# ecmwf/earthkit-meteo

Measured on NVIDIA B200. Metric: thermo grid-points/s, higher is better.
Workload: dtype f64

## Files before the change

### earthkit-meteo_b200/csrc/ek_api.cu

```cuda
#include <cstring>
#include <vector>

#include "ek_launch.cuh"

namespace ek {

std::atomic<int> g_ctas_per_sm{16};
std::atomic<uint64_t> g_launches{0};

static thread_local char t_err[512] = "";

int set_error(int code, const char* fmt, ...) {
    va_list ap;
    va_start(ap, fmt);
    vsnprintf(t_err, sizeof(t_err), fmt, ap);
    va_end(ap);
    return code;
}

int sm_count_current_device() {
    static std::atomic<int> cache[64];
    int dev = -1;
    if (cudaGetDevice(&dev) != cudaSuccess || dev < 0) return -1;
    if (dev < 64) {
        int v = cache[dev].load(std::memory_order_relaxed);
        if (v > 0) return v;
    }
    int sms = 0;
    if (cudaDeviceGetAttribute(&sms, cudaDevAttrMultiProcessorCount, dev) != cudaSuccess) return -1;
    if (dev < 64) cache[dev].store(sms, std::memory_order_relaxed);
    return sms;
}

}

using namespace ek;

extern "C" EK_EXPORT int ek_thermo_version(void) { return EK_THERMO_VERSION; }
extern "C" EK_EXPORT const char* ek_thermo_last_error(void) { return t_err; }
extern "C" EK_EXPORT uint64_t ek_thermo_launch_count(void) { return g_launches.load(std::memory_order_relaxed); }

extern "C" EK_EXPORT int ek_thermo_set_launch_config(int threads, int ctas_per_sm) {
    if (threads != 0 && threads != kThreads) return set_error(EK_ERR_ARG, "threads=%d: the CTA size is fixed at build time (%d)", threads, kThreads);
    if (ctas_per_sm != 0) {
        if (ctas_per_sm < 1 || ctas_per_sm > 4096) return set_error(EK_ERR_ARG, "ctas_per_sm=%d out of range", ctas_per_sm);
        g_ctas_per_sm.store(ctas_per_sm);
    }
    return EK_OK;
}

extern "C" EK_EXPORT int ek_thermo_shard_range(int64_t n, int world, int rank, int64_t align, int64_t* begin, int64_t* end) {
    if (n < 0 || world < 1 || rank < 0 || rank >= world || align < 1 || !begin || !end)
        return set_error(EK_ERR_ARG, "shard_range: bad arguments n=%lld world=%d rank=%d align=%lld", (long long)n, world, rank, (long long)align);
    const int64_t units = n / align;
    const int64_t base = units / world, extra = units % world;
    const int64_t b = (rank * base + (rank < extra ? rank : extra)) * align;
    int64_t e = b + (base + (rank < extra ? 1 : 0)) * align;
    if (rank == world - 1) e = n;
    *begin = b;
    *end = e;
    return EK_OK;
}

template <typename T> int ek_suite_launch_tqp(const ek_operand* ins, void* const* outs, uint32_t mask, int ept_method, int64_t n, void* stream);
template <typename T> int ek_suite_launch_ttdp(const ek_operand* ins, void* const* outs, uint32_t mask, int ept_method, int64_t n, void* stream);
template <typename T>
int ek_suite_launch_hybrid(const void* t, const void* q, const void* sp, const void* A, const void* B, int nlev, int64_t npl, void* const* outs,
                           uint32_t out_mask, int ept_method, void* stream);

namespace {
struct StreamSet {
    std::vector<cudaStream_t> s;
    ~StreamSet() {
        for (auto st : s) cudaStreamSynchronize(st);
        for (auto st : s) cudaStreamDestroy(st);
    }
    int create(int n) {
        for (int i = 0; i < n; ++i) {
            cudaStream_t st;
            cudaError_t e = cudaStreamCreateWithFlags(&st, cudaStreamNonBlocking);
            if (e != cudaSuccess) return set_error((int)e, "host pipeline: cudaStreamCreate: %s", cudaGetErrorString(e));
            s.push_back(st);
        }
        return EK_OK;
    }
    int drain() {
        for (auto st : s) {
            cudaError_t e = cudaStreamSynchronize(st);
            if (e != cudaSuccess) return set_error((int)e, "host pipeline: stream sync: %s", cudaGetErrorString(e));
        }
        return EK_OK;
    }
};

int count_outputs(const char* what, void* const* h_outs, uint32_t out_mask, int* n_out) {
    if (out_mask == 0 || out_mask >= (1u << S_NSLOTS)) return set_error(EK_ERR_ARG, "%s: out_mask=0x%x", what, out_mask);
    *n_out = 0;
    for (int k = 0; k < S_NSLOTS; ++k)
        if ((out_mask >> k) & 1u) {
            if (!h_outs[k]) return set_error(EK_ERR_ARG, "%s: output %d requested but its buffer is NULL", what, k);
// ... 132 lines not shown
```

### earthkit-meteo_b200/csrc/ek_launch.cuh

```cuda
#pragma once
#include <atomic>
#include <cstdarg>
#include <cstdio>

#include "../../include/ek_thermo.h"
#include "ek_thermo_kernels.cuh"

#define EK_EXPORT __attribute__((visibility("default")))

#ifndef EK_SMALL_WAVE_SPARE
#define EK_SMALL_WAVE_SPARE 0
#endif

namespace ek {

int set_error(int code, const char* fmt, ...);
int sm_count_current_device();
extern std::atomic<int> g_ctas_per_sm;
extern std::atomic<uint64_t> g_launches;

inline bool aligned16(const void* p) { return (reinterpret_cast<uintptr_t>(p) & 15u) == 0; }

template <typename T> constexpr unsigned smem_for() { return sizeof(T) == 8 ? kSmemBytes : 0u; }

template <auto Kernel> inline void prepare_smem(unsigned smem_bytes) {
    if (smem_bytes == 0) return;
    static std::atomic<uint64_t> done{0};
    int dev = 0;
    if (cudaGetDevice(&dev) != cudaSuccess || dev < 0) return;
    const uint64_t bit = dev < 64 ? (1ull << dev) : 0;
    if (bit && (done.load(std::memory_order_relaxed) & bit)) return;
    const unsigned want = EK_MIN_CTAS * (smem_bytes + 1024u);
    int pct = (int)((want * 100u + 228u * 1024u - 1u) / (228u * 1024u));
    if (pct > 100) pct = 100;
    cudaFuncSetAttribute(Kernel, cudaFuncAttributePreferredSharedMemoryCarveout, pct);
    if (smem_bytes > 48u * 1024u) cudaFuncSetAttribute(Kernel, cudaFuncAttributeMaxDynamicSharedMemorySize, (int)smem_bytes);
    if (bit) done.fetch_or(bit, std::memory_order_relaxed);
}

template <auto Kernel, typename... Args> inline void launch_kernel_smem(int blocks, cudaStream_t st, unsigned smem, Args... args) {
    prepare_smem<Kernel>(smem);
    Kernel<<<blocks, kThreads, smem, st>>>(args...);
}
template <auto Kernel, typename T, typename... Args> inline void launch_kernel(int blocks, cudaStream_t st, Args... args) {
    launch_kernel_smem<Kernel>(blocks, st, smem_for<T>(), args...);
}

template <auto Kernel, typename... Args>
inline void launch_streaming(unsigned blocks, unsigned smem, cudaStream_t st, Args... args) {
    prepare_smem<Kernel>(smem);
    cudaLaunchConfig_t cfg = {};
    cfg.gridDim = dim3(blocks);
    cfg.blockDim = dim3(kThreads);
    cfg.dynamicSmemBytes = smem;
    cfg.stream = st;
    cudaLaunchAttribute attr[1];
    attr[0].id = cudaLaunchAttributeProgrammaticStreamSerialization;
    attr[0].val.programmaticStreamSerializationAllowed = 1;
    cfg.attrs = attr;
    cfg.numAttrs = EK_PDL ? 1 : 0;
    cudaLaunchKernelEx(&cfg, Kernel, args...);
}

template <class Op, class OpE, typename T>
int launch(const char* what, const ek_operand* ins, void* const* outs, int64_t n, Params P, void* stream) {
    if (n < 0) return set_error(EK_ERR_ARG, "%s: n=%lld must be >= 0", what, (long long)n);
    InArgs<Op::NIN> in;
    OutArgs<Op::NOUT> out;
    int vec_ok = 1;
    for (int k = 0; k < Op::NIN; ++k) {
        in.p[k] = ins[k].ptr;
        in.s[k] = ins[k].value;
        if (ins[k].ptr) {
            if (!aligned16(ins[k].ptr)) vec_ok = 0;
            if (reinterpret_cast<uintptr_t>(ins[k].ptr) % sizeof(T))
                return set_error(EK_ERR_ARG, "%s: input %d is not aligned to its element size", what, k);
        }
    }
    uint32_t mask = 0;
    for (int o = 0; o < Op::NOUT; ++o) {
        out.p[o] = outs[o];
        if (outs[o]) {
            mask |= 1u << o;
            if (!aligned16(outs[o])) vec_ok = 0;
            if (reinterpret_cast<uintptr_t>(outs[o]) % sizeof(T))
                return set_error(EK_ERR_ARG, "%s: output %d is not aligned to its element size", what, o);
        }
    }
    if (mask == 0) return set_error(EK_ERR_ARG, "%s: no output buffer given", what);
    P.out_mask = mask;
    if (n == 0) return EK_OK;

    constexpr int threads = kThreads;
    constexpr int unroll = UnrollOf<Op>::value;
    const int64_t tile = (int64_t)threads * Vec16<T>::N * unroll;
    const int64_t ntiles = n / tile;
    const int64_t tail_blocks = ((n - ntiles * tile) + threads - 1) / threads;
    const int sms = sm_count_current_device();
    if (sms <= 0) return set_error(EK_ERR_ARG, "%s: no CUDA device is current", what);
    int64_t cap = (int64_t)sms * g_ctas_per_sm.load(std::memory_order_relaxed);
    const int64_t wave = (int64_t)sms * (MinCtasOf<Op>::value - EK_SMALL_WAVE_SPARE);
    if (ntiles <= 8 * wave && wave < cap) cap = wave;
    int64_t blocks = ntiles > tail_blocks ? ntiles : tail_blocks;
    if (blocks > cap) blocks = cap;
    if (blocks < 1) blocks = 1;

    launch_streaming<&ew_kernel<Op, OpE, T, unroll>>((unsigned)blocks, smem_for<T>(), static_cast<cudaStream_t>(stream), in, out, n, P, vec_ok);
    g_launches.fetch_add(1, std::memory_order_relaxed);
    cudaError_t err = cudaGetLastError();
    if (err != cudaSuccess) return set_error((int)err, "%s: kernel launch failed: %s", what, cudaGetErrorString(err));
    return EK_OK;
}

template <class Op, class OpE, typename T>
int launch_batch(const char* what, int n_seg, const void* const* const* ins, const double* scalars, const double* last_scalars,
                 void* const* const* outs, int64_t n_per_seg, Params P, void* stream) {
    if (n_seg < 0 || n_per_seg < 0) return set_error(EK_ERR_ARG, "%s: n_seg=%d n_per_seg=%lld", what, n_seg, (long long)n_per_seg);
    uint32_t in_mask = 0, out_mask = 0;
    for (int k = 0; k < Op::NIN; ++k)
        if (ins[k]) in_mask |= 1u << k;
    for (int o = 0; o < Op::NOUT; ++o)
        if (outs[o]) out_mask |= 1u << o;
    if (out_mask == 0) return set_error(EK_ERR_ARG, "%s: no output buffer given", what);
    if (last_scalars && ins[Op::NIN - 1]) return set_error(EK_ERR_ARG, "%s: the last input is given both as fields and as per-segment scalars", what);
    P.out_mask = out_mask;
    if (n_seg == 0 || n_per_seg == 0) return EK_OK;
    const int sms = sm_count_current_device();
    if (sms <= 0) return set_error(EK_ERR_ARG, "%s: no CUDA device is current", what);
    constexpr int unroll = UnrollOf<Op>::value;
    const int64_t tile = (int64_t)kThreads * Vec16<T>::N * unroll;
    for (int s0 = 0; s0 < n_seg; s0 += kBatchMaxSeg) {
        BatchArgs<Op::NIN, Op::NOUT> B;
        B.n_seg = n_seg - s0 < kBatchMaxSeg ? n_seg - s0 : kBatchMaxSeg;
        B.in_mask = in_mask;
        B.out_mask = out_mask;
        B.last_per_seg = last_scalars ? 1 : 0;
        for (int j = 0; j < B.n_seg; ++j) B.s_last[j] = last_scalars ? last_scalars[s0 + j] : 0.0;
        int vec_ok = 1;
        for (int k = 0; k < Op::NIN; ++k) {
            B.s[k] = scalars ? scalars[k] : 0.0;
            for (int j = 0; j < B.n_seg; ++j) {
                B.in[k][j] = ins[k] ? ins[k][s0 + j] : nullptr;
                if (ins[k]) {
                    if (!B.in[k][j] || reinterpret_cast<uintptr_t>(B.in[k][j]) % sizeof(T))
                        return set_error(EK_ERR_ARG, "%s: input %d of segment %d is NULL or not aligned to its element size", what, k, s0 + j);
                    if (!aligned16(B.in[k][j])) vec_ok = 0;
                }
            }
        }
        for (int o = 0; o < Op::NOUT; ++o)
            for (int j = 0; j < B.n_seg; ++j) {
                B.out[o][j] = outs[o] ? outs[o][s0 + j] : nullptr;
                if (outs[o]) {
                    if (!B.out[o][j] || reinterpret_cast<uintptr_t>(B.out[o][j]) % sizeof(T))
                        return set_error(EK_ERR_ARG, "%s: output %d of segment %d is NULL or not aligned to its element size", what, o, s0 + j);
                    if (!aligned16(B.out[o][j])) vec_ok = 0;
                }
            }
        const int64_t ntiles = (n_per_seg / tile) * B.n_seg;
        const int64_t tail_blocks = ((n_per_seg % tile) * B.n_seg + kThreads - 1) / kThreads;
        int64_t cap = (int64_t)sms * g_ctas_per_sm.load(std::memory_order_relaxed);
        const int64_t wave = (int64_t)sms * MinCtasOf<Op>::value;
        if (ntiles <= 8 * wave && wave < cap) cap = wave;
        int64_t blocks = ntiles > tail_blocks ? ntiles : tail_blocks;
        if (blocks > cap) blocks = cap;
        if (blocks < 1) blocks = 1;
        launch_streaming<&ew_batch_kernel<Op, OpE, T, unroll>>((unsigned)blocks, smem_for<T>(), static_cast<cudaStream_t>(stream), B, n_per_seg, P, vec_ok);
        g_launches.fetch_add(1, std::memory_order_relaxed);
        cudaError_t err = cudaGetLastError();
        if (err != cudaSuccess) return set_error((int)err, "%s: kernel launch failed: %s", what, cudaGetErrorString(err));
    }
    return EK_OK;
}

inline bool valid_phase(int v) { return v >= 0 && v <= 2; }

#define EK_API(NAME, PARAMS, ARGS)                                                    \
    extern "C" EK_EXPORT int ek_thermo_##NAME##_f64 PARAMS { return impl_##NAME<double> ARGS; } \
    extern "C" EK_EXPORT int ek_thermo_##NAME##_f32 PARAMS { return impl_##NAME<float> ARGS; }

}
```

### earthkit-meteo_b200/csrc/ek_thermo_kernels.cuh

```cuda
#pragma once
#include <cuda_runtime.h>

#include "ek_thermo_math.cuh"

#ifndef EK_UNROLL
#define EK_UNROLL 2
#endif
#ifndef EK_PIPELINE
#define EK_PIPELINE 0
#endif
#ifndef EK_MAX_THREADS
#define EK_MAX_THREADS 256
#endif
#ifndef EK_DEFER_TILE
#define EK_DEFER_TILE 0
#endif
#ifndef EK_PF_DIST
#define EK_PF_DIST 2
#endif
#ifndef EK_HEAVY_MIN_CTAS
#define EK_HEAVY_MIN_CTAS 3
#endif
#ifndef EK_LAST_SCALAR_LOOP
#define EK_LAST_SCALAR_LOOP 1
#endif
#ifndef EK_PDL
#define EK_PDL 1
#endif
#ifndef EK_MIN_CTAS
#define EK_MIN_CTAS 4
#endif

namespace ek {

template <int N> struct InArgs {
    const void* p[N];
    double s[N];
};
template <int N> struct OutArgs {
    void* p[N];
};

template <typename T> struct Vec16;
template <> struct Vec16<double> {
    using type = double2;
    static constexpr int N = 2;
    static __device__ __forceinline__ void load(const double* src, double* dst) {
        double2 v = __ldcs(reinterpret_cast<const double2*>(src));
        dst[0] = v.x;
        dst[1] = v.y;
    }
    static __device__ __forceinline__ void store(double* dst, const double* src) {
        __stcs(reinterpret_cast<double2*>(dst), make_double2(src[0], src[1]));
    }
};
template <> struct Vec16<float> {
    using type = float4;
    static constexpr int N = 4;
    static __device__ __forceinline__ void load(const float* src, float* dst) {
        float4 v = __ldcs(reinterpret_cast<const float4*>(src));
        dst[0] = v.x;
        dst[1] = v.y;
        dst[2] = v.z;
        dst[3] = v.w;
    }
    static __device__ __forceinline__ void store(float* dst, const float* src) {
        __stcs(reinterpret_cast<float4*>(dst), make_float4(src[0], src[1], src[2], src[3]));
    }
};

#if EK_LEAN_MATH
constexpr unsigned kSmemBytes = 2 * 8 * EK_LOG_TAB_N + 8 * EK_EXP_TAB_N;
#else
constexpr unsigned kSmemBytes = 0;
#endif

constexpr int kThreads = EK_MAX_THREADS;

template <typename T> __device__ __forceinline__ bool is_nan_val(T v) { return v != v; }

template <class OpE, typename T> __device__ __noinline__ void cold_point(const T* a, T* r, const Params P, const uint32_t array_mask) {
    bool missing = array_mask != 0;
#pragma unroll
    for (int k = 0; k < OpE::NIN; ++k)
        if ((array_mask >> k) & 1u) missing = missing && is_nan_val(a[k]);
    if (missing) return;
#pragma unroll
    for (int o = 0; o < OpE::NOUT; ++o) r[o] = T(0);
    OpE::template apply<T>(a, r, P);
}

template <int NOUT> __device__ __forceinline__ bool any_nan(const double* r) {
    int m = 0;
#pragma unroll
    for (int o = 0; o < NOUT; ++o) m = max(m, __double2hiint(r[o]) & 0x7fffffff);
    return m >= 0x7ff80000;
}
template <int NOUT> __device__ __forceinline__ bool any_nan(const float* r) {
    int m = 0;
#pragma unroll
    for (int o = 0; o < NOUT; ++o) m = max(m, __float_as_int(r[o]) & 0x7fffffff);
    return m > 0x7f800000;
}

template <class Op, class = void> struct ColdF32 {
    static constexpr bool value = false;
};
template <class Op> struct ColdF32<Op, decltype((void)Op::COLD_F32)> {
    static constexpr bool value = Op::COLD_F32;
};

template <class Op, class OpE, typename T>
__device__ __forceinline__ void point(const T* a, T* r, const Params& P, const uint32_t array_mask) {
#pragma unroll
    for (int o = 0; o < Op::NOUT; ++o) r[o] = T(0);
    Op::template apply<T>(a, r, P);
#if EK_LEAN_DEVICE
    if ((sizeof(T) == 8 || ColdF32<Op>::value) && __builtin_expect(any_nan<Op::NOUT>(r), 0)) {
        T a2[Op::NIN], r2[Op::NOUT];
#pragma unroll
// ... 234 lines not shown
                } else {
#pragma unroll
                    for (int v = 0; v < VEC; ++v) __stcs(dst + v, y[o][v]);
                }
            }
        }
    }
}

template <class Op, class OpE, typename T, int UNROLL, bool VECOK, int ALLARR>
__device__ __forceinline__ void tile_loop(const InArgs<Op::NIN>& in, const OutArgs<Op::NOUT>& out, const int64_t ntiles, const Params& P,
                                          const uint32_t array_mask) {
    constexpr int TILE = kThreads * Vec16<T>::N * UNROLL;
    const int64_t G = gridDim.x;
    const int64_t toff = (int64_t)threadIdx.x * Vec16<T>::N;
    int64_t ta = blockIdx.x;
    if (ta >= ntiles) return;
#if EK_PIPELINE
    TileRegs<Op, T, UNROLL> A, B;
    load_tile<Op, T, UNROLL, VECOK, ALLARR>(A, in, ta * TILE + toff);
    for (;;) {
        const int64_t tb = ta + G;
        const bool hb = tb < ntiles;
        if (hb) load_tile<Op, T, UNROLL, VECOK, ALLARR>(B, in, tb * TILE + toff);
        compute_store_tile<Op, OpE, T, UNROLL, VECOK>(A, out, ta * TILE + toff, P, array_mask);
        if (!hb) break;
        ta = tb + G;
        const bool ha = ta < ntiles;
        if (ha) load_tile<Op, T, UNROLL, VECOK, ALLARR>(A, in, ta * TILE + toff);
        compute_store_tile<Op, OpE, T, UNROLL, VECOK>(B, out, tb * TILE + toff, P, array_mask);
        if (!ha) break;
    }
#else
    for (; ta < ntiles; ta += G) {
        TileRegs<Op, T, UNROLL> A;
        load_tile<Op, T, UNROLL, VECOK, ALLARR>(A, in, ta * TILE + toff);
        if (Op::PREFETCH_NEXT && ta + EK_PF_DIST * G < ntiles) prefetch_tile_l2<Op, T, UNROLL>(in, (ta + EK_PF_DIST * G) * TILE + toff);
        compute_store_tile<Op, OpE, T, UNROLL, VECOK>(A, out, ta * TILE + toff, P, array_mask);
    }
#endif
}

__device__ __forceinline__ void pdl_release() {
#if EK_PDL
    asm volatile("griddepcontrol.launch_dependents;");
#endif
}
__device__ __forceinline__ void pdl_acquire() {
#if EK_PDL
    asm volatile("griddepcontrol.wait;" ::: "memory");
#endif
}

template <class Op, class OpE, typename T, int UNROLL>
__global__ void __launch_bounds__(kThreads, MinCtasOf<Op>::value)
    ew_kernel(const InArgs<Op::NIN> in, const OutArgs<Op::NOUT> out, const int64_t n, const Params P, const int vec_ok) {
    constexpr int NIN = Op::NIN;
    constexpr int NOUT = Op::NOUT;
    constexpr int TILE = kThreads * Vec16<T>::N * UNROLL;
    pdl_release();
#if EK_LEAN_DEVICE
    static_assert(sizeof(lean::Tables) == kSmemBytes, "kSmemBytes must match lean::Tables");
    if (sizeof(T) == 8) lean::init_tables();
#endif
    pdl_acquire();
    const int64_t ntiles = n / TILE;
    uint32_t array_mask = 0;
#pragma unroll
    for (int k = 0; k < NIN; ++k) array_mask |= (in.p[k] != nullptr) ? (1u << k) : 0u;
    if (vec_ok && array_mask == (1u << NIN) - 1u)
        tile_loop<Op, OpE, T, UNROLL, true, 1>(in, out, ntiles, P, array_mask);
    else if (LastScalarLoopOf<Op>::value && NIN >= 2 && vec_ok && array_mask == (1u << (NIN - 1)) - 1u)
        tile_loop<Op, OpE, T, UNROLL, true, 2>(in, out, ntiles, P, array_mask);
    else if (vec_ok)
        tile_loop<Op, OpE, T, UNROLL, true, 0>(in, out, ntiles, P, array_mask);
    else
        tile_loop<Op, OpE, T, UNROLL, false, 0>(in, out, ntiles, P, array_mask);

    for (int64_t i = ntiles * TILE + (int64_t)blockIdx.x * kThreads + threadIdx.x; i < n; i += (int64_t)gridDim.x * kThreads) {
        T a[NIN], r[NOUT];
#pragma unroll
        for (int k = 0; k < NIN; ++k) a[k] = (in.p[k] != nullptr) ? __ldcs(static_cast<const T*>(in.p[k]) + i) : static_cast<T>(in.s[k]);
        point<Op, OpE, T>(a, r, P, array_mask);
#pragma unroll
        for (int o = 0; o < NOUT; ++o) {
            const bool w = Op::STATIC_MASK ? (((Op::STATIC_MASK >> o) & 1u) != 0) : (out.p[o] != nullptr);
            if (w) __stcs(static_cast<T*>(out.p[o]) + i, r[o]);
        }
    }
}

constexpr int kBatchMaxSeg = 128;
template <int NIN, int NOUT> struct BatchArgs {
    const void* in[NIN][kBatchMaxSeg];
    void* out[NOUT][kBatchMaxSeg];
    double s[NIN];
    double s_last[kBatchMaxSeg];
    int last_per_seg;
    uint32_t in_mask;
    uint32_t out_mask;
    int n_seg;
};

template <class Op, class OpE, typename T, int UNROLL>
__global__ void __launch_bounds__(kThreads, MinCtasOf<Op>::value)
    ew_batch_kernel(const __grid_constant__ BatchArgs<Op::NIN, Op::NOUT> B, const int64_t n_per_seg, const Params P, const int vec_ok) {
    constexpr int NIN = Op::NIN;
    constexpr int NOUT = Op::NOUT;
    constexpr int TILE = kThreads * Vec16<T>::N * UNROLL;
    pdl_release();
#if EK_LEAN_DEVICE
    if (sizeof(T) == 8) lean::init_tables();
#endif
    pdl_acquire();
    const int64_t tiles_per_seg = n_per_seg / TILE;
    const int64_t ntiles = tiles_per_seg * B.n_seg;
    const int64_t toff = (int64_t)threadIdx.x * Vec16<T>::N;
    const bool all_arrays = B.in_mask == (1u << NIN) - 1u;
    for (int64_t tile = blockIdx.x; tile < ntiles; tile += gridDim.x) {
        const int seg = (int)(tile / tiles_per_seg);
        const int64_t base = (tile - (int64_t)seg * tiles_per_seg) * TILE + toff;
        InArgs<NIN> in;
        OutArgs<NOUT> out;
#pragma unroll
        for (int k = 0; k < NIN; ++k) {
            in.p[k] = ((B.in_mask >> k) & 1u) ? B.in[k][seg] : nullptr;
            in.s[k] = (k == NIN - 1 && B.last_per_seg) ? B.s_last[seg] : B.s[k];
        }
#pragma unroll
        for (int o = 0; o < NOUT; ++o) out.p[o] = ((B.out_mask >> o) & 1u) ? B.out[o][seg] : nullptr;
        auto prefetch_next = [&]() {
            if (Op::PREFETCH_NEXT) {
                const int64_t nt = tile + EK_PF_DIST * (int64_t)gridDim.x;
                if (nt < ntiles) {
                    const int nseg = (int)(nt / tiles_per_seg);
                    InArgs<NIN> nin;
    #pragma unroll
                    for (int k = 0; k < NIN; ++k) nin.p[k] = ((B.in_mask >> k) & 1u) ? B.in[k][nseg] : nullptr;
                    prefetch_tile_l2<Op, T, UNROLL>(nin, (nt - (int64_t)nseg * tiles_per_seg) * TILE + toff);
                }
            }
        };
// ... 40 lines not shown
```

### earthkit-meteo_b200/csrc/ek_thermo_ops.inc

```
#ifndef EK_EPT_HEAVY
#define EK_EPT_HEAVY 1
#endif
#ifndef EK_EPT_PREFETCH
#define EK_EPT_PREFETCH 1
#endif
#ifndef EK_SUITE_UNROLL
#define EK_SUITE_UNROLL 0
#endif

namespace ek {
namespace EK_MODE_NS {

#undef EK_OP_BEGIN
#undef EK_OP_END
#define EK_OP_BEGIN(NAME, NIN_, NOUT_)                                               \
    struct NAME {                                                                    \
        static constexpr int NIN = NIN_;                                             \
        static constexpr int NOUT = NOUT_;                                           \
        static constexpr uint32_t STATIC_MASK = (1u << NOUT_) - 1u;                  \
        static constexpr bool PREFETCH_NEXT = false;                                 \
        template <typename T> static EK_HD void apply(const T* in, T* out, const Params& P) {
#define EK_OP_END \
    }             \
    }             \
// ... 91 lines not shown
        for (int j = 0; j < N; ++j) {
            ept[j] = P.opt0 ? ept_from_q_point<M>(in[j][0], in[j][1], in[j][2]) : ept_point<M>(in[j][0], in[j][1], T(0), false, in[j][2]);
            p[j] = P.opt1 ? CK(p0) : in[j][2];
        }
        t_on_ma_n<M, TM>(ept, p, tw);
        for (int j = 0; j < N; ++j) {
            out[j][0] = ept[j];
            out[j][1] = tw[j];
        }
    }
};
template <int M, int TM> struct OpTOnMa {
    static constexpr int NIN = 2;
    static constexpr int NOUT = 1;
    static constexpr uint32_t STATIC_MASK = 1;
    static constexpr bool PREFETCH_NEXT = false;
    static constexpr bool COLD_F32 = (TM == TM_BISECT);
    static constexpr int UNROLL = (TM == TM_NEWTON) ? 1 : 0;
    template <typename T> static EK_HD void apply(const T* in, T* out, const Params&) {
        out[0] = t_on_ma<M, TM>(in[0], in[1]);
    }
    static constexpr bool BATCH = (TM == TM_BISECT);
    template <typename T, int N> static EK_HD void apply_n(const T (&in)[N][NIN], T (&out)[N][NOUT], const Params&) {
        T ept[N], p[N], tw[N];
        for (int j = 0; j < N; ++j) ept[j] = in[j][0], p[j] = in[j][1];
        t_on_ma_n<M, TM>(ept, p, tw);
        for (int j = 0; j < N; ++j) out[j][0] = tw[j];
    }
};
template <int M> struct OpSatEpt {
    static constexpr int NIN = 2;
    static constexpr int NOUT = 1;
    static constexpr uint32_t STATIC_MASK = 1;
    static constexpr bool PREFETCH_NEXT = false;
    template <typename T> static EK_HD void apply(const T* in, T* out, const Params&) {
        out[0] = sat_ept_point<M>(in[0], in[1]);
    }
};


#ifndef EK_SUITE_PREFETCH_MIN
#define EK_SUITE_PREFETCH_MIN 2
#endif
constexpr int suite_popcount(uint32_t m) { return m == 0 ? 0 : (int)(m & 1u) + suite_popcount(m >> 1); }

#ifndef EK_GENERIC_SUITE_LAST_SCALAR
#define EK_GENERIC_SUITE_LAST_SCALAR 0
#endif
template <uint32_t MASK, int M> struct OpSuiteTQPm {
    static constexpr int NIN = 3;
    static constexpr int NOUT = S_NSLOTS;
    static constexpr uint32_t STATIC_MASK = MASK;
    static constexpr bool HEAVY = true;
    static constexpr int UNROLL = EK_SUITE_UNROLL;
    static constexpr bool PREFETCH_NEXT = MASK == 0 || suite_popcount(MASK) >= EK_SUITE_PREFETCH_MIN;
    static constexpr bool LAST_SCALAR_LOOP = MASK != 0 || EK_GENERIC_SUITE_LAST_SCALAR;
    template <typename T> static EK_HD void apply(const T* in, T* out, const Params& P) {
        const uint32_t m = MASK ? MASK : P.out_mask;
        constexpr uint32_t EPT = (1u << S_EPT) | (1u << S_WBPT);
        const T t = in[0], q = in[1], p = in[2];
        T th = T(0), tvf = T(0), e = T(0), td = T(0), w = T(0);
        if (m & ((1u << S_THETA) | (1u << S_THETAV))) th = theta(t, p);
        if (m & ((1u << S_TV) | (1u << S_THETAV))) tvf = tv_factor(q);
        if (m & ((1u << S_RH) | (1u << S_TDQ) | (1u << S_E) | EPT)) e = e_from_q(q, p);
        if (m & (1u << S_THETA)) out[S_THETA] = th;
        if (m & ((1u << S_ES) | (1u << S_RH))) {
            T es = es_mixed(t);
            out[S_ES] = es;
            if (m & (1u << S_RH)) out[S_RH] = m_div(T(100.0) * e, es);
        }
        if (m & ((1u << S_TDQ) | EPT)) td = t_from_es(e);
        if (m & (1u << S_TDQ)) out[S_TDQ] = td;
        if (m & (1u << S_TV)) out[S_TV] = t * tvf;
        if ((m & (1u << S_W)) || ((m & EPT) && M != EPT_IFS)) w = w_from_q(q);
        if (m & (1u << S_W)) out[S_W] = w;
        if (m & (1u << S_E)) out[S_E] = e;
        if (m & (1u << S_THETAV)) out[S_THETAV] = th * tvf;
        if (m & EPT) {
            const T ept = ept_core<M>(t, td, M == EPT_IFS ? q : w, p);
            if (m & (1u << S_EPT)) out[S_EPT] = ept;
            if (m & (1u << S_WBPT)) out[S_WBPT] = wbpt_direct(ept);
        }
    }
};

template <uint32_t MASK, int M> struct OpSuiteTTdPm {
    static constexpr int NIN = 3;
    static constexpr int NOUT = S_NSLOTS;
    static constexpr uint32_t STATIC_MASK = MASK;
    static constexpr bool HEAVY = true;
    static constexpr int UNROLL = EK_SUITE_UNROLL;
    static constexpr bool PREFETCH_NEXT = MASK == 0 || suite_popcount(MASK) >= EK_SUITE_PREFETCH_MIN;
    static constexpr bool LAST_SCALAR_LOOP = MASK != 0 || EK_GENERIC_SUITE_LAST_SCALAR;
    template <typename T> static EK_HD void apply(const T* in, T* out, const Params& P) {
        const uint32_t m = MASK ? MASK : P.out_mask;
        constexpr uint32_t EPT = (1u << S_EPT) | (1u << S_WBPT);
        const T t = in[0], td = in[1], p = in[2];
        T th = T(0), e = T(0), q = T(0), w = T(0);
        if (m & ((1u << S_THETA) | (1u << S_THETAV))) th = theta(t, p);
        if (m & ((1u << S_RH) | (1u << S_TDQ) | (1u << S_TV) | (1u << S_W) | (1u << S_E) | (1u << S_THETAV) | EPT)) e = es_water(td);
        if ((m & ((1u << S_TDQ) | (1u << S_TV) | (1u << S_THETAV))) || ((m & EPT) && M == EPT_IFS)) q = q_from_e(e, p, CK(eps_default));
        if (m & (1u << S_THETA)) out[S_THETA] = th;
        if ((m & (1u << S_ES)) && (m & (1u << S_RH))) {
            const T ew = es_water(t);
            out[S_ES] = es_mixed_given_water(t, ew);
            out[S_RH] = m_div(T(100.0) * e, ew);
        } else {
            if (m & (1u << S_ES)) out[S_ES] = es_mixed(t);
            if (m & (1u << S_RH)) out[S_RH] = m_div(T(100.0) * e, es_water(t));
        }
        if (m & (1u << S_TDQ)) out[S_TDQ] = q;
        if (m & (1u << S_TV)) out[S_TV] = t * tv_factor(q);
        if ((m & (1u << S_W)) || ((m & EPT) && M != EPT_IFS)) w = w_from_e(e, p, CK(eps_default));
        if (m & (1u << S_W)) out[S_W] = w;
        if (m & (1u << S_E)) out[S_E] = e;
        if (m & (1u << S_THETAV)) out[S_THETAV] = th * tv_factor(q);
        if (m & EPT) {
            const T ept = ept_core<M>(t, td, M == EPT_IFS ? q : w, p);
            if (m & (1u << S_EPT)) out[S_EPT] = ept;
            if (m & (1u << S_WBPT)) out[S_WBPT] = wbpt_direct(ept);
        }
    }
};

using OpSuiteTQP = OpSuiteTQPm<0, EPT_IFS>;
using OpSuiteTTdP = OpSuiteTTdPm<0, EPT_IFS>;

}
}
```

### earthkit-meteo_b200/ek_thermo/_backend.py

```python
from __future__ import annotations

import ctypes
import os
from ctypes import c_double, c_int, c_int64, c_size_t, c_uint32, c_uint64, c_void_p

import torch

_HERE = os.path.dirname(os.path.abspath(__file__))
LIB_NAME = os.environ.get("EK_THERMO_LIB", "libek_thermo.so")
LIB_PATH = LIB_NAME if os.path.isabs(LIB_NAME) else os.path.join(_HERE, LIB_NAME)


class ek_operand(ctypes.Structure):

    _fields_ = [("ptr", c_void_p), ("value", c_double)]


class EkThermoError(RuntimeError):
    pass


if not os.path.exists(LIB_PATH):
    raise ImportError(
        f"ek_thermo: CUDA library {LIB_PATH} not found. Build it with `python -c 'import __graft_entry__ as g; g.build()'` "
        "or `make -C earthkit-meteo_b200/csrc`. There is no CPU fallback."
    )
_lib = ctypes.CDLL(LIB_PATH)
_lib.ek_thermo_version.restype = c_int
_lib.ek_thermo_last_error.restype = ctypes.c_char_p
_lib.ek_thermo_launch_count.restype = c_uint64
_lib.ek_thermo_set_launch_config.argtypes = [c_int, c_int]
_lib.ek_thermo_shard_range.argtypes = [c_int64, c_int, c_int, c_int64, ctypes.POINTER(c_int64), ctypes.POINTER(c_int64)]

_SUFFIX = {torch.float64: "f64", torch.float32: "f32"}

SIGNATURES = {
    "celsius_to_kelvin": (1, (), 1),
    "kelvin_to_celsius": (1, (), 1),
    "specific_humidity_from_mixing_ratio": (1, (), 1),
    "mixing_ratio_from_specific_humidity": (1, (), 1),
    "vapour_pressure_from_specific_humidity": (2, (), 1),
    "vapour_pressure_from_mixing_ratio": (2, (), 1),
    "specific_humidity_from_vapour_pressure": (2, (c_double,), 1),
    "mixing_ratio_from_vapour_pressure": (2, (c_double,), 1),
    "saturation_vapour_pressure": (1, (c_int,), 1),
    "saturation_vapour_pressure_slope": (1, (c_int,), 1),
    "saturation_mixing_ratio": (2, (c_int,), 1),
    "saturation_specific_humidity": (2, (c_int,), 1),
    "saturation_mixing_ratio_slope": (4, (c_int, c_int, c_int, c_double), 1),
    "saturation_specific_humidity_slope": (4, (c_int, c_int, c_int, c_double), 1),
    "temperature_from_saturation_vapour_pressure": (1, (), 1),
    "relative_humidity_from_dewpoint": (2, (), 1),
    "relative_humidity_from_specific_humidity": (3, (), 1),
    "specific_humidity_from_dewpoint": (2, (), 1),
    "mixing_ratio_from_dewpoint": (2, (), 1),
    "specific_humidity_from_relative_humidity": (3, (), 1),
    "dewpoint_from_relative_humidity": (2, (), 1),
    "dewpoint_from_specific_humidity": (2, (), 1),
    "virtual_temperature": (2, (), 1),
    "virtual_potential_temperature": (3, (), 1),
    "potential_temperature": (2, (), 1),
    "temperature_from_potential_temperature": (2, (), 1),
    "pressure_on_dry_adiabat": (3, (), 1),
    "temperature_on_dry_adiabat": (3, (), 1),
    "lcl_temperature": (2, (c_int,), 1),
    "lcl": (3, (c_int,), 2),
    "specific_gas_constant": (1, (), 1),
    "ept_from_dewpoint": (3, (c_int,), 1),
    "ept_from_specific_humidity": (3, (c_int,), 1),
    "saturation_ept": (2, (c_int,), 1),
    "temperature_on_moist_adiabat": (2, (c_int, c_int), 1),
    "wet_bulb_temperature_from_dewpoint": (3, (c_int, c_int), 1),
    "wet_bulb_temperature_from_specific_humidity": (3, (c_int, c_int), 1),
    "wet_bulb_potential_temperature_from_dewpoint": (3, (c_int, c_int), 1),
    "wet_bulb_potential_temperature_from_specific_humidity": (3, (c_int, c_int), 1),
    "ept_wet_bulb": (3, (c_int, c_int, c_int, c_int), 2),
    "wind_speed": (2, (), 1),
    "wind_direction": (2, (c_int, c_int), 1),
    "wind_xy_to_polar": (2, (c_int,), 2),
    "wind_polar_to_xy": (2, (c_int,), 2),
    "w_from_omega": (3, (), 1),
    "coriolis": (1, (), 1),
    "height_from_thickness": (2, (c_int,), 1),
}
# ... 1 lines not shown
for _name, (_nin, _opts, _nout) in SIGNATURES.items():
    for _sfx in ("f64", "f32"):
        _fn = getattr(_lib, f"ek_thermo_{_name}_{_sfx}")
        _fn.argtypes = [ek_operand] * _nin + list(_opts) + [c_void_p] * _nout + [c_int64, c_void_p]
        _fn.restype = c_int
for _name in ("suite_tqp", "suite_ttdp"):
    for _sfx in ("f64", "f32"):
        _fn = getattr(_lib, f"ek_thermo_{_name}_{_sfx}")
        _fn.argtypes = [ek_operand] * 3 + [ctypes.POINTER(c_void_p), c_uint32, c_int, c_int64, c_void_p]
        _fn.restype = c_int
for _name in ("suite_tqp_batch", "suite_ttdp_batch"):
    for _sfx in ("f64", "f32"):
        _fn = getattr(_lib, f"ek_thermo_{_name}_{_sfx}")
        _fn.argtypes = [c_int, c_void_p, c_void_p, c_void_p, ctypes.POINTER(c_double), ctypes.POINTER(c_double), ctypes.POINTER(c_void_p), c_uint32, c_int,
                        c_int64, c_void_p]
        _fn.restype = c_int
_c_int_p = ctypes.POINTER(c_int)
for _sfx in ("f64", "f32"):
    _fn = getattr(_lib, f"ek_thermo_pressure_on_hybrid_levels_{_sfx}")
    _fn.argtypes = [c_void_p, c_void_p, c_int, c_void_p, c_int64, c_void_p, c_int, c_void_p, c_int, c_int, c_int, c_double,
                    c_void_p, c_void_p, c_void_p, c_void_p, c_int, c_void_p]
    _fn.restype = c_int
    _fn = getattr(_lib, f"ek_thermo_hybrid_top_is_toa_{_sfx}")
    _fn.argtypes = [c_void_p, c_int64, c_double, c_double, c_void_p, c_void_p]
    _fn.restype = c_int
    _fn = getattr(_lib, f"ek_thermo_geopotential_on_hybrid_levels_{_sfx}")
    _fn.argtypes = [c_void_p, c_void_p, c_int, c_int64, c_void_p, c_void_p, c_void_p, c_int, c_int, c_double, c_void_p, c_void_p, c_void_p,
                    c_int, c_void_p, c_void_p]
    _fn.restype = c_int
    _fn = getattr(_lib, f"ek_thermo_suite_tq_hybrid_{_sfx}")
    _fn.argtypes = [c_void_p, c_void_p, c_void_p, c_void_p, c_void_p, c_int, c_int64, ctypes.POINTER(c_void_p), c_uint32, c_int, c_void_p,
                    c_void_p]
    _fn.restype = c_int
for _sfx in ("f64", "f32"):
    _fn = getattr(_lib, f"ek_thermo_host_suite_{_sfx}")
    _fn.argtypes = [c_int, c_void_p, c_void_p, c_void_p, ctypes.POINTER(c_void_p), c_uint32, c_int, c_int64, c_void_p, c_size_t, c_int]
    _fn.restype = c_int
    _fn = getattr(_lib, f"ek_thermo_host_suite_tq_hybrid_{_sfx}")
    _fn.argtypes = [c_void_p, c_void_p, c_void_p, c_void_p, c_void_p, c_int, c_int64, ctypes.POINTER(c_void_p), c_uint32, c_int, c_void_p,
                    c_size_t, c_int]
    _fn.restype = c_int


def version() -> int:
    return int(_lib.ek_thermo_version())


def launch_count() -> int:
    return int(_lib.ek_thermo_launch_count())


def set_launch_config(threads: int = 0, ctas_per_sm: int = 0) -> None:
    _check(_lib.ek_thermo_set_launch_config(threads, ctas_per_sm))


def _check(rc: int) -> None:
    if rc == 0:
        return
    msg = (_lib.ek_thermo_last_error() or b"").decode()
    if rc == -3:
        raise ValueError(msg)
    if rc < 0:
        raise ValueError(f"ek_thermo: {msg} (code {rc})")
    raise EkThermoError(f"ek_thermo: {msg} (cudaError {rc})")


def _check_device(tensors):
    dev = None
    for t in tensors:
        if not t.is_cuda:
            raise TypeError(
                "ek_thermo: got a CPU tensor. This package only runs on CUDA tensors (no CPU fallback); "
                "use earthkit.meteo.thermo for host arrays."
            )
        if dev is None:
            dev = t.device
        elif t.device != dev:
            raise ValueError(f"ek_thermo: tensors are on different devices ({dev} and {t.device})")
    return dev


_Tensor = torch.Tensor


def _on_device(t):
    return t.is_cuda


def _prepare(args):
    first = None
    ops = []
    for a in args:
        if isinstance(a, _Tensor):
            if first is None:
                first = a
                dtype = a.dtype
                shape = a.shape
                dev = a.device
                if dtype not in _SUFFIX:
                    return _prepare_general(args)
            elif a.dtype != dtype or a.shape != shape or a.device != dev:
                return _prepare_general(args)
            if not a.is_contiguous():
                return _prepare_general(args)
            ops.append(ek_operand(a.data_ptr(), 0.0))
        elif type(a) is float:
# ... 240 lines not shown
```

### include/ek_thermo.h

```cpp
#ifndef EK_THERMO_H
#define EK_THERMO_H

#include <stddef.h>
#include <stdint.h>

#ifdef __cplusplus
extern "C" {
#endif

#define EK_THERMO_VERSION 111

typedef struct ek_operand {
    const void* ptr;
    double value;
} ek_operand;

enum { EK_OK = 0, EK_ERR_ARG = -1, EK_ERR_ENUM = -2, EK_ERR_EPS = -3, EK_ERR_PIPE = -4 };

enum { EK_PHASE_MIXED = 0, EK_PHASE_WATER = 1, EK_PHASE_ICE = 2 };
enum { EK_LCL_DAVIES = 0, EK_LCL_BOLTON = 1 };
enum { EK_EPT_IFS = 0, EK_EPT_BOLTON35 = 1, EK_EPT_BOLTON39 = 2 };
enum { EK_TM_NONE = 0, EK_TM_DIRECT = 1, EK_TM_BISECT = 2, EK_TM_NEWTON = 3 };
enum { EK_HUM_DEWPOINT = 0, EK_HUM_SPECIFIC = 1 };

enum {
    EK_S_THETA = 0, EK_S_ES = 1, EK_S_RH = 2, EK_S_TD_OR_Q = 3, EK_S_TV = 4, EK_S_W = 5, EK_S_E = 6, EK_S_THETAV = 7,
    EK_S_EPT = 8,
    EK_S_WBPT = 9,
    EK_S_NSLOTS = 10
};

#define EK_THERMO_FN(name, ...)              \
    int ek_thermo_##name##_f64(__VA_ARGS__); \
    int ek_thermo_##name##_f32(__VA_ARGS__);

int ek_thermo_version(void);
const char* ek_thermo_last_error(void);
int ek_thermo_set_launch_config(int threads, int ctas_per_sm);
uint64_t ek_thermo_launch_count(void);
int ek_thermo_shard_range(int64_t n, int world, int rank, int64_t align, int64_t* begin, int64_t* end);

EK_THERMO_FN(celsius_to_kelvin, ek_operand t, void* out, int64_t n, void* stream)
EK_THERMO_FN(kelvin_to_celsius, ek_operand t, void* out, int64_t n, void* stream)
EK_THERMO_FN(specific_humidity_from_mixing_ratio, ek_operand w, void* out, int64_t n, void* stream)
EK_THERMO_FN(mixing_ratio_from_specific_humidity, ek_operand q, void* out, int64_t n, void* stream)
EK_THERMO_FN(vapour_pressure_from_specific_humidity, ek_operand q, ek_operand p, void* out, int64_t n, void* stream)
EK_THERMO_FN(vapour_pressure_from_mixing_ratio, ek_operand w, ek_operand p, void* out, int64_t n, void* stream)
EK_THERMO_FN(specific_humidity_from_vapour_pressure, ek_operand e, ek_operand p, double eps, void* out, int64_t n, void* stream)
EK_THERMO_FN(mixing_ratio_from_vapour_pressure, ek_operand e, ek_operand p, double eps, void* out, int64_t n, void* stream)

EK_THERMO_FN(saturation_vapour_pressure, ek_operand t, int phase, void* out, int64_t n, void* stream)
EK_THERMO_FN(saturation_vapour_pressure_slope, ek_operand t, int phase, void* out, int64_t n, void* stream)
EK_THERMO_FN(saturation_mixing_ratio, ek_operand t, ek_operand p, int phase, void* out, int64_t n, void* stream)
EK_THERMO_FN(saturation_specific_humidity, ek_operand t, ek_operand p, int phase, void* out, int64_t n, void* stream)
EK_THERMO_FN(saturation_mixing_ratio_slope, ek_operand t, ek_operand p, ek_operand es, ek_operand es_slope, int has_es,
             int has_es_slope, int phase, double eps, void* out, int64_t n, void* stream)
EK_THERMO_FN(saturation_specific_humidity_slope, ek_operand t, ek_operand p, ek_operand es, ek_operand es_slope, int has_es,
             int has_es_slope, int phase, double eps, void* out, int64_t n, void* stream)
EK_THERMO_FN(temperature_from_saturation_vapour_pressure, ek_operand es, void* out, int64_t n, void* stream)

EK_THERMO_FN(relative_humidity_from_dewpoint, ek_operand t, ek_operand td, void* out, int64_t n, void* stream)
EK_THERMO_FN(relative_humidity_from_specific_humidity, ek_operand t, ek_operand q, ek_operand p, void* out, int64_t n, void* stream)
EK_THERMO_FN(specific_humidity_from_dewpoint, ek_operand td, ek_operand p, void* out, int64_t n, void* stream)
EK_THERMO_FN(mixing_ratio_from_dewpoint, ek_operand td, ek_operand p, void* out, int64_t n, void* stream)
EK_THERMO_FN(specific_humidity_from_relative_humidity, ek_operand t, ek_operand r, ek_operand p, void* out, int64_t n, void* stream)
EK_THERMO_FN(dewpoint_from_relative_humidity, ek_operand t, ek_operand r, void* out, int64_t n, void* stream)
EK_THERMO_FN(dewpoint_from_specific_humidity, ek_operand q, ek_operand p, void* out, int64_t n, void* stream)

EK_THERMO_FN(virtual_temperature, ek_operand t, ek_operand q, void* out, int64_t n, void* stream)
EK_THERMO_FN(virtual_potential_temperature, ek_operand t, ek_operand q, ek_operand p, void* out, int64_t n, void* stream)
EK_THERMO_FN(potential_temperature, ek_operand t, ek_operand p, void* out, int64_t n, void* stream)
EK_THERMO_FN(temperature_from_potential_temperature, ek_operand th, ek_operand p, void* out, int64_t n, void* stream)
EK_THERMO_FN(pressure_on_dry_adiabat, ek_operand t, ek_operand t_def, ek_operand p_def, void* out, int64_t n, void* stream)
EK_THERMO_FN(temperature_on_dry_adiabat, ek_operand p, ek_operand t_def, ek_operand p_def, void* out, int64_t n, void* stream)
EK_THERMO_FN(lcl_temperature, ek_operand t, ek_operand td, int method, void* out, int64_t n, void* stream)
EK_THERMO_FN(lcl, ek_operand t, ek_operand td, ek_operand p, int method, void* t_lcl_out, void* p_lcl_out, int64_t n, void* stream)
EK_THERMO_FN(specific_gas_constant, ek_operand q, void* out, int64_t n, void* stream)

EK_THERMO_FN(ept_from_dewpoint, ek_operand t, ek_operand td, ek_operand p, int method, void* out, int64_t n, void* stream)
EK_THERMO_FN(ept_from_specific_humidity, ek_operand t, ek_operand q, ek_operand p, int method, void* out, int64_t n, void* stream)
EK_THERMO_FN(saturation_ept, ek_operand t, ek_operand p, int method, void* out, int64_t n, void* stream)
EK_THERMO_FN(temperature_on_moist_adiabat, ek_operand ept, ek_operand p, int ept_method, int t_method, void* out, int64_t n, void* stream)
EK_THERMO_FN(wet_bulb_temperature_from_dewpoint, ek_operand t, ek_operand td, ek_operand p, int ept_method, int t_method, void* out,
             int64_t n, void* stream)
EK_THERMO_FN(wet_bulb_temperature_from_specific_humidity, ek_operand t, ek_operand q, ek_operand p, int ept_method, int t_method,
             void* out, int64_t n, void* stream)
EK_THERMO_FN(wet_bulb_potential_temperature_from_dewpoint, ek_operand t, ek_operand td, ek_operand p, int ept_method, int t_method,
             void* out, int64_t n, void* stream)
EK_THERMO_FN(wet_bulb_potential_temperature_from_specific_humidity, ek_operand t, ek_operand q, ek_operand p, int ept_method,
             int t_method, void* out, int64_t n, void* stream)

// ... 41 lines not shown
```

Before: 93.06 billion.

## Stage suite outputs in shared memory and write them with TMA bulk stores

Adds a per-warp tile loop for the compile-time suite kernels with up to five outputs. Each warp computes its outputs into a shared-memory slice, and lane 0 then issues cp.async.bulk global stores in place of per-thread streaming vector stores. The aim is to cut store instruction count and make output writes asynchronous with the next tile's loads and compute. In exchange it uses more dynamic shared memory per CTA, which can lower occupancy, and adds async-proxy fences and bulk wait_group sync. It applies only to large, aligned, all-array launches and can be switched off at runtime.

```diff
diff --git a/earthkit-meteo_b200/csrc/ek_api.cu b/earthkit-meteo_b200/csrc/ek_api.cu
--- a/earthkit-meteo_b200/csrc/ek_api.cu
+++ b/earthkit-meteo_b200/csrc/ek_api.cu
@@ -7,6 +7,7 @@
 
 std::atomic<int> g_ctas_per_sm{16};
 std::atomic<uint64_t> g_launches{0};
+std::atomic<int> g_bulk_store{1};
 
 static thread_local char t_err[512] = "";
 
@@ -46,6 +47,12 @@
         if (ctas_per_sm < 1 || ctas_per_sm > 4096) return set_error(EK_ERR_ARG, "ctas_per_sm=%d out of range", ctas_per_sm);
         g_ctas_per_sm.store(ctas_per_sm);
     }
+    return EK_OK;
+}
+
+extern "C" EK_EXPORT int ek_thermo_set_bulk_store(int enable) {
+    if (enable && !EK_BULK_STORE) return set_error(EK_ERR_ARG, "set_bulk_store: this library is built without bulk stores (EK_BULK_STORE=0)");
+    g_bulk_store.store(enable ? 1 : 0);
     return EK_OK;
 }
 
diff --git a/earthkit-meteo_b200/csrc/ek_launch.cuh b/earthkit-meteo_b200/csrc/ek_launch.cuh
--- a/earthkit-meteo_b200/csrc/ek_launch.cuh
+++ b/earthkit-meteo_b200/csrc/ek_launch.cuh
@@ -2,6 +2,7 @@
 #include <atomic>
 #include <cstdarg>
 #include <cstdio>
+#include <mutex>
 
 #include "../../include/ek_thermo.h"
 #include "ek_thermo_kernels.cuh"
@@ -18,24 +19,25 @@
 int sm_count_current_device();
 extern std::atomic<int> g_ctas_per_sm;
 extern std::atomic<uint64_t> g_launches;
+extern std::atomic<int> g_bulk_store;
 
 inline bool aligned16(const void* p) { return (reinterpret_cast<uintptr_t>(p) & 15u) == 0; }
 
-template <typename T> constexpr unsigned smem_for() { return sizeof(T) == 8 ? kSmemBytes : 0u; }
-
-template <auto Kernel> inline void prepare_smem(unsigned smem_bytes) {
+template <auto Kernel> inline void prepare_smem(unsigned smem_bytes, int ctas_per_sm = EK_MIN_CTAS) {
     if (smem_bytes == 0) return;
-    static std::atomic<uint64_t> done{0};
+    static std::atomic<unsigned> done[64];
+    static std::mutex mu;
     int dev = 0;
     if (cudaGetDevice(&dev) != cudaSuccess || dev < 0) return;
-    const uint64_t bit = dev < 64 ? (1ull << dev) : 0;
-    if (bit && (done.load(std::memory_order_relaxed) & bit)) return;
-    const unsigned want = EK_MIN_CTAS * (smem_bytes + 1024u);
+    if (dev < 64 && done[dev].load(std::memory_order_acquire) >= smem_bytes) return;
+    std::lock_guard<std::mutex> lock(mu);
+    if (dev < 64 && done[dev].load(std::memory_order_relaxed) >= smem_bytes) return;
+    const unsigned want = (unsigned)ctas_per_sm * (smem_bytes + 1024u);
     int pct = (int)((want * 100u + 228u * 1024u - 1u) / (228u * 1024u));
     if (pct > 100) pct = 100;
     cudaFuncSetAttribute(Kernel, cudaFuncAttributePreferredSharedMemoryCarveout, pct);
     if (smem_bytes > 48u * 1024u) cudaFuncSetAttribute(Kernel, cudaFuncAttributeMaxDynamicSharedMemorySize, (int)smem_bytes);
-    if (bit) done.fetch_or(bit, std::memory_order_relaxed);
+    if (dev < 64) done[dev].store(smem_bytes, std::memory_order_release);
 }
 
 template <auto Kernel, typename... Args> inline void launch_kernel_smem(int blocks, cudaStream_t st, unsigned smem, Args... args) {
@@ -47,11 +49,10 @@
 }
 
 template <auto Kernel, typename... Args>
-inline void launch_streaming(unsigned blocks, unsigned smem, cudaStream_t st, Args... args) {
-    prepare_smem<Kernel>(smem);
+inline void launch_streaming(unsigned blocks, unsigned threads, unsigned smem, cudaStream_t st, Args... args) {
     cudaLaunchConfig_t cfg = {};
     cfg.gridDim = dim3(blocks);
-    cfg.blockDim = dim3(kThreads);
+    cfg.blockDim = dim3(threads);
     cfg.dynamicSmemBytes = smem;
     cfg.stream = st;
     cudaLaunchAttribute attr[1];
@@ -100,12 +101,23 @@
     if (sms <= 0) return set_error(EK_ERR_ARG, "%s: no CUDA device is current", what);
     int64_t cap = (int64_t)sms * g_ctas_per_sm.load(std::memory_order_relaxed);
     const int64_t wave = (int64_t)sms * (MinCtasOf<Op>::value - EK_SMALL_WAVE_SPARE);
-    if (ntiles <= 8 * wave && wave < cap) cap = wave;
+    const bool small = ntiles <= 8 * wave;
+    if (small && wave < cap) cap = wave;
     int64_t blocks = ntiles > tail_blocks ? ntiles : tail_blocks;
     if (blocks > cap) blocks = cap;
     if (blocks < 1) blocks = 1;
 
-    launch_streaming<&ew_kernel<Op, OpE, T, unroll>>((unsigned)blocks, smem_for<T>(), static_cast<cudaStream_t>(stream), in, out, n, P, vec_ok);
+    unsigned smem = smem_for<T>();
+    if constexpr (BulkStoreOf<Op>::value) {
+        bool all_arrays = true;
+        for (int k = 0; k < Op::NIN; ++k) all_arrays = all_arrays && in.p[k] != nullptr;
+        if (!small && vec_ok && all_arrays && g_bulk_store.load(std::memory_order_relaxed)) {
+            vec_ok = 2;
+            smem = bulk_store_smem_bytes<Op, T>();
+        }
+    }
+    prepare_smem<&ew_kernel<Op, OpE, T, unroll>>(smem);
+    launch_streaming<&ew_kernel<Op, OpE, T, unroll>>((unsigned)blocks, kThreads, smem, static_cast<cudaStream_t>(stream), in, out, n, P, vec_ok);
     g_launches.fetch_add(1, std::memory_order_relaxed);
     cudaError_t err = cudaGetLastError();
     if (err != cudaSuccess) return set_error((int)err, "%s: kernel launch failed: %s", what, cudaGetErrorString(err));
@@ -165,7 +177,8 @@
         int64_t blocks = ntiles > tail_blocks ? ntiles : tail_blocks;
         if (blocks > cap) blocks = cap;
         if (blocks < 1) blocks = 1;
-        launch_streaming<&ew_batch_kernel<Op, OpE, T, unroll>>((unsigned)blocks, smem_for<T>(), static_cast<cudaStream_t>(stream), B, n_per_seg, P, vec_ok);
+        prepare_smem<&ew_batch_kernel<Op, OpE, T, unroll>>(smem_for<T>());
+        launch_streaming<&ew_batch_kernel<Op, OpE, T, unroll>>((unsigned)blocks, kThreads, smem_for<T>(), static_cast<cudaStream_t>(stream), B, n_per_seg, P, vec_ok);
         g_launches.fetch_add(1, std::memory_order_relaxed);
         cudaError_t err = cudaGetLastError();
         if (err != cudaSuccess) return set_error((int)err, "%s: kernel launch failed: %s", what, cudaGetErrorString(err));
diff --git a/earthkit-meteo_b200/csrc/ek_thermo_kernels.cuh b/earthkit-meteo_b200/csrc/ek_thermo_kernels.cuh
--- a/earthkit-meteo_b200/csrc/ek_thermo_kernels.cuh
+++ b/earthkit-meteo_b200/csrc/ek_thermo_kernels.cuh
@@ -52,6 +52,11 @@
     }
     static __device__ __forceinline__ void store(double* dst, const double* src) {
         __stcs(reinterpret_cast<double2*>(dst), make_double2(src[0], src[1]));
+    }
+    static __device__ __forceinline__ void load_shared(const double* src, double* dst) {
+        const double2 v = *reinterpret_cast<const double2*>(src);
+        dst[0] = v.x;
+        dst[1] = v.y;
     }
 };
 template <> struct Vec16<float> {
@@ -66,6 +71,13 @@
     }
     static __device__ __forceinline__ void store(float* dst, const float* src) {
         __stcs(reinterpret_cast<float4*>(dst), make_float4(src[0], src[1], src[2], src[3]));
+    }
+    static __device__ __forceinline__ void load_shared(const float* src, float* dst) {
+        const float4 v = *reinterpret_cast<const float4*>(src);
+        dst[0] = v.x;
+        dst[1] = v.y;
+        dst[2] = v.z;
+        dst[3] = v.w;
     }
 };
 
@@ -406,11 +418,116 @@
 #endif
 }
 
+template <class Op, class OpE, typename T>
+__device__ __forceinline__ void tail_points(const InArgs<Op::NIN>& in, const OutArgs<Op::NOUT>& out, int64_t i, const int64_t n, const int64_t step,
+                                            const Params& P, const uint32_t array_mask) {
+    for (; i < n; i += step) {
+        T a[Op::NIN], r[Op::NOUT];
+#pragma unroll
+        for (int k = 0; k < Op::NIN; ++k) a[k] = (in.p[k] != nullptr) ? __ldcs(static_cast<const T*>(in.p[k]) + i) : static_cast<T>(in.s[k]);
+        point<Op, OpE, T>(a, r, P, array_mask);
+#pragma unroll
+        for (int o = 0; o < Op::NOUT; ++o) {
+            const bool w = Op::STATIC_MASK ? (((Op::STATIC_MASK >> o) & 1u) != 0) : (out.p[o] != nullptr);
+            if (w) __stcs(static_cast<T*>(out.p[o]) + i, r[o]);
+        }
+    }
+}
+
+#ifndef EK_BULK_STORE
+#define EK_BULK_STORE 1
+#endif
+
+template <class Op, class = void> struct BulkStoreOf {
+    static constexpr bool value = false;
+};
+template <class Op> struct BulkStoreOf<Op, decltype((void)Op::BULK_STORE)> {
+    static constexpr bool value = EK_BULK_STORE != 0 && Op::BULK_STORE;
+};
+
+__host__ __device__ constexpr int popcount_u32(uint32_t m) { return m == 0 ? 0 : (int)(m & 1u) + popcount_u32(m >> 1); }
+
+template <typename T> __host__ __device__ constexpr unsigned smem_for() { return sizeof(T) == 8 ? kSmemBytes : 0u; }
+template <class Op, typename T> __host__ __device__ constexpr unsigned bulk_store_smem_bytes() {
+    return smem_for<T>() + (unsigned)((kThreads / 32) * popcount_u32(Op::STATIC_MASK) * 32 * Vec16<T>::N * UnrollOf<Op>::value * sizeof(T));
+}
+
+template <class Op, class OpE, typename T, int UNROLL>
+__device__ __forceinline__ void tile_loop_bulk_store(const InArgs<Op::NIN>& in, const OutArgs<Op::NOUT>& out, const int64_t ntiles,
+                                                     const Params& P, const uint32_t array_mask) {
+    constexpr int NIN = Op::NIN;
+    constexpr int NOUT = Op::NOUT;
+    constexpr uint32_t MASK = Op::STATIC_MASK;
+    constexpr int VEC = Vec16<T>::N;
+    constexpr int TILE = kThreads * VEC * UNROLL;
+    constexpr int SLICE = 32 * VEC * UNROLL;
+    constexpr uint32_t SLICE_BYTES = SLICE * sizeof(T);
+    static_assert(MASK != 0 && !IsBatch<Op>::value && !DeferColdOf<Op>::value, "the bulk-store loop is for the suites' compile-time output sets");
+    extern __shared__ __align__(16) unsigned char ek_smem_raw[];
+    const int warp = threadIdx.x / 32, lane = threadIdx.x % 32;
+    T* buf = reinterpret_cast<T*>(ek_smem_raw + smem_for<T>()) + warp * popcount_u32(MASK) * SLICE;
+    const uint32_t buf_s = static_cast<uint32_t>(__cvta_generic_to_shared(buf));
+    const int64_t woff = (int64_t)warp * SLICE;
+    for (int64_t ta = blockIdx.x; ta < ntiles; ta += gridDim.x) {
+        const int64_t base = ta * TILE + woff;
+        TileRegs<Op, T, UNROLL> A;
+#pragma unroll
+        for (int k = 0; k < NIN; ++k)
+#pragma unroll
+            for (int u = 0; u < UNROLL; ++u) Vec16<T>::load(static_cast<const T*>(in.p[k]) + base + u * 32 * VEC + lane * VEC, A.x[k][u]);
+        if (Op::PREFETCH_NEXT && ta + EK_PF_DIST * gridDim.x < ntiles) {
+            const int64_t nb = (ta + EK_PF_DIST * gridDim.x) * TILE + woff + lane * VEC;
+#pragma unroll
+            for (int k = 0; k < NIN; ++k)
+#pragma unroll
+                for (int u = 0; u < UNROLL; ++u) asm volatile("prefetch.global.L2 [%0];" ::"l"(static_cast<const T*>(in.p[k]) + nb + u * 32 * VEC));
+        }
+        if (lane == 0) asm volatile("cp.async.bulk.wait_group.read 0;" ::: "memory");
+        __syncwarp();
+#pragma unroll
+        for (int u = 0; u < UNROLL; ++u) {
+            T y[NOUT][VEC];
+#pragma unroll
+            for (int v = 0; v < VEC; ++v) {
+                T a[NIN], res[NOUT];
+#pragma unroll
+                for (int k = 0; k < NIN; ++k) a[k] = A.x[k][u][v];
+                point<Op, OpE, T>(a, res, P, array_mask);
+#pragma unroll
+                for (int o = 0; o < NOUT; ++o) y[o][v] = res[o];
+            }
+            int j = 0;
+#pragma unroll
+            for (int o = 0; o < NOUT; ++o)
+                if ((MASK >> o) & 1u) {
+                    T* d = buf + j * SLICE + u * 32 * VEC + lane * VEC;
+#pragma unroll
+                    for (int v = 0; v < VEC; ++v) d[v] = y[o][v];
+                    ++j;
+                }
+        }
+        asm volatile("fence.proxy.async.shared::cta;" ::: "memory");
+        __syncwarp();
+        if (lane == 0) {
+            int j = 0;
+#pragma unroll
+            for (int o = 0; o < NOUT; ++o)
+                if ((MASK >> o) & 1u) {
+                    asm volatile("cp.async.bulk.global.shared::cta.bulk_group [%0], [%1], %2;" ::"l"(static_cast<T*>(out.p[o]) + base),
+                                 "r"(buf_s + j * SLICE_BYTES), "r"(SLICE_BYTES)
+                                 : "memory");
+                    ++j;
+                }
+            asm volatile("cp.async.bulk.commit_group;" ::: "memory");
+        }
+    }
+    if (lane == 0) asm volatile("cp.async.bulk.wait_group 0;" ::: "memory");
+}
+
 template <class Op, class OpE, typename T, int UNROLL>
 __global__ void __launch_bounds__(kThreads, MinCtasOf<Op>::value)
     ew_kernel(const InArgs<Op::NIN> in, const OutArgs<Op::NOUT> out, const int64_t n, const Params P, const int vec_ok) {
     constexpr int NIN = Op::NIN;
-    constexpr int NOUT = Op::NOUT;
     constexpr int TILE = kThreads * Vec16<T>::N * UNROLL;
     pdl_release();
 #if EK_LEAN_DEVICE
@@ -422,6 +539,14 @@
     uint32_t array_mask = 0;
 #pragma unroll
     for (int k = 0; k < NIN; ++k) array_mask |= (in.p[k] != nullptr) ? (1u << k) : 0u;
+    if constexpr (BulkStoreOf<Op>::value) {
+        if (vec_ok == 2) {
+            tile_loop_bulk_store<Op, OpE, T, UNROLL>(in, out, ntiles, P, array_mask);
+            tail_points<Op, OpE, T>(in, out, ntiles * TILE + (int64_t)blockIdx.x * kThreads + threadIdx.x, n, (int64_t)gridDim.x * kThreads, P,
+                                    array_mask);
+            return;
+        }
+    }
     if (vec_ok && array_mask == (1u << NIN) - 1u)
         tile_loop<Op, OpE, T, UNROLL, true, 1>(in, out, ntiles, P, array_mask);
     else if (LastScalarLoopOf<Op>::value && NIN >= 2 && vec_ok && array_mask == (1u << (NIN - 1)) - 1u)
@@ -431,17 +556,7 @@
     else
         tile_loop<Op, OpE, T, UNROLL, false, 0>(in, out, ntiles, P, array_mask);
 
-    for (int64_t i = ntiles * TILE + (int64_t)blockIdx.x * kThreads + threadIdx.x; i < n; i += (int64_t)gridDim.x * kThreads) {
-        T a[NIN], r[NOUT];
-#pragma unroll
-        for (int k = 0; k < NIN; ++k) a[k] = (in.p[k] != nullptr) ? __ldcs(static_cast<const T*>(in.p[k]) + i) : static_cast<T>(in.s[k]);
-        point<Op, OpE, T>(a, r, P, array_mask);
-#pragma unroll
-        for (int o = 0; o < NOUT; ++o) {
-            const bool w = Op::STATIC_MASK ? (((Op::STATIC_MASK >> o) & 1u) != 0) : (out.p[o] != nullptr);
-            if (w) __stcs(static_cast<T*>(out.p[o]) + i, r[o]);
-        }
-    }
+    tail_points<Op, OpE, T>(in, out, ntiles * TILE + (int64_t)blockIdx.x * kThreads + threadIdx.x, n, (int64_t)gridDim.x * kThreads, P, array_mask);
 }
 
 constexpr int kBatchMaxSeg = 128;
diff --git a/earthkit-meteo_b200/csrc/ek_thermo_ops.inc b/earthkit-meteo_b200/csrc/ek_thermo_ops.inc
--- a/earthkit-meteo_b200/csrc/ek_thermo_ops.inc
+++ b/earthkit-meteo_b200/csrc/ek_thermo_ops.inc
@@ -167,6 +167,7 @@
     static constexpr int NOUT = S_NSLOTS;
     static constexpr uint32_t STATIC_MASK = MASK;
     static constexpr bool HEAVY = true;
+    static constexpr bool BULK_STORE = MASK != 0 && suite_popcount(MASK) <= 5;
     static constexpr int UNROLL = EK_SUITE_UNROLL;
     static constexpr bool PREFETCH_NEXT = MASK == 0 || suite_popcount(MASK) >= EK_SUITE_PREFETCH_MIN;
     static constexpr bool LAST_SCALAR_LOOP = MASK != 0 || EK_GENERIC_SUITE_LAST_SCALAR;
@@ -204,6 +205,7 @@
     static constexpr int NOUT = S_NSLOTS;
     static constexpr uint32_t STATIC_MASK = MASK;
     static constexpr bool HEAVY = true;
+    static constexpr bool BULK_STORE = MASK != 0 && suite_popcount(MASK) <= 5;
     static constexpr int UNROLL = EK_SUITE_UNROLL;
     static constexpr bool PREFETCH_NEXT = MASK == 0 || suite_popcount(MASK) >= EK_SUITE_PREFETCH_MIN;
     static constexpr bool LAST_SCALAR_LOOP = MASK != 0 || EK_GENERIC_SUITE_LAST_SCALAR;
diff --git a/earthkit-meteo_b200/ek_thermo/_backend.py b/earthkit-meteo_b200/ek_thermo/_backend.py
--- a/earthkit-meteo_b200/ek_thermo/_backend.py
+++ b/earthkit-meteo_b200/ek_thermo/_backend.py
@@ -30,6 +30,7 @@
 _lib.ek_thermo_last_error.restype = ctypes.c_char_p
 _lib.ek_thermo_launch_count.restype = c_uint64
 _lib.ek_thermo_set_launch_config.argtypes = [c_int, c_int]
+_lib.ek_thermo_set_bulk_store.argtypes = [c_int]
 _lib.ek_thermo_shard_range.argtypes = [c_int64, c_int, c_int, c_int64, ctypes.POINTER(c_int64), ctypes.POINTER(c_int64)]
 
 _SUFFIX = {torch.float64: "f64", torch.float32: "f32"}
@@ -137,6 +138,10 @@
 
 def set_launch_config(threads: int = 0, ctas_per_sm: int = 0) -> None:
     _check(_lib.ek_thermo_set_launch_config(threads, ctas_per_sm))
+
+
+def set_bulk_store(enable: bool) -> None:
+    _check(_lib.ek_thermo_set_bulk_store(1 if enable else 0))
 
 
 def _check(rc: int) -> None:
diff --git a/include/ek_thermo.h b/include/ek_thermo.h
--- a/include/ek_thermo.h
+++ b/include/ek_thermo.h
@@ -8,7 +8,7 @@
 extern "C" {
 #endif
 
-#define EK_THERMO_VERSION 111
+#define EK_THERMO_VERSION 112
 
 typedef struct ek_operand {
     const void* ptr;
@@ -37,6 +37,7 @@
 int ek_thermo_version(void);
 const char* ek_thermo_last_error(void);
 int ek_thermo_set_launch_config(int threads, int ctas_per_sm);
+int ek_thermo_set_bulk_store(int enable);
 uint64_t ek_thermo_launch_count(void);
 int ek_thermo_shard_range(int64_t n, int world, int rank, int64_t align, int64_t* begin, int64_t* end);
 
```

New measurement: 91.80 billion, median of 6. 1.4% lower.
